# levi106/kvedge

Measured on AMD Instinct MI355X. Metric: images/sec ResNet-50 edge module at 1/2/4/8 MI355X; VM boot-to-ready sec, higher is better.
Workload: dtype bf16; 1 GPU; model=resnet50, global_batch=1280, per_gpu_batch=1280, image_size=224, parallelism=dp1, backend=none, hip_graph=True, streams=2, microbatch=0, mb_blocks=3

## Files before the change

### csrc/bindings/ops.cpp

```cpp
#include <ATen/ATen.h>
#include <c10/core/DeviceGuard.h>
#include <c10/hip/HIPStream.h>
#include <torch/library.h>

#include "../kernels/kvedge_kernels.h"

namespace {

hipStream_t cur_stream(const at::Tensor& t) {
  return c10::hip::getCurrentHIPStream(t.device().index()).stream();
}

void check_dev(const at::Tensor& t, const char* name) {
  TORCH_CHECK(t.is_cuda(), "kvedge: ", name, " must be a GPU tensor");
  TORCH_CHECK(t.is_contiguous(), "kvedge: ", name, " must be contiguous");
}

void check_bf16(const at::Tensor& t, const char* name) {
  check_dev(t, name);
  TORCH_CHECK(t.scalar_type() == at::kBFloat16, "kvedge: ", name, " must be bf16");
}

void set_splitk_ws(KvConvParams& p, const at::Tensor& ws) {
  p.ws = ws.data_ptr<float>();
// ... 78 lines not shown
  p.x = x.data_ptr();
  p.w = w.data_ptr();
  p.bias = bias.data_ptr<float>();
  p.N = (int)N; p.H = (int)H; p.W = (int)W; p.Cin = (int)Cin;
  p.ldx = (int)ldx; p.x_coff = (int)x_coff;
  p.Ho = (int)H; p.Wo = (int)W; p.Cout = (int)Cout;
  p.KH = 3; p.KW = 3; p.stride = 1; p.pad = 1;
  p.K = (int)(9 * Cin); p.Kpad = (int)w.size(1);
  p.M = (int)(N * H * W);
  p.act = (int)act; p.mode = 0;
  p.w_t = w2.data_ptr(); p.bias_t = b2.data_ptr<float>(); p.z = z.data_ptr();
  p.n_t = (int)C2; p.ldz = (int)z.size(3); p.z_coff = (int)z_coff;
  p.pair_1x1 = 1;
  const int rc = kv_conv_pair(&p, (int)tile, cur_stream(x));
  TORCH_CHECK(rc == 0, "kvedge: conv_pair failed rc=", rc);
}

void conv_dual(const at::Tensor& x1, const at::Tensor& x2, const at::Tensor& w,
               const c10::optional<at::Tensor>& bias, at::Tensor& y, int64_t stride2,
               int64_t act, int64_t tile, const c10::optional<at::Tensor>& ws) {
  check_bf16(x1, "x1");
  check_bf16(x2, "x2");
  check_bf16(w, "w");
  check_bf16(y, "y");
  TORCH_CHECK(x1.dim() == 4 && x2.dim() == 4 && y.dim() == 4, "kvedge: NHWC tensors");
  const int64_t N = x1.size(0), Ho = x1.size(1), Wo = x1.size(2), K1 = x1.size(3);
  const int64_t K2 = x2.size(3), Cout = y.size(3);
  TORCH_CHECK(x2.size(0) == N && (x2.size(1) + stride2 - 1) / stride2 == Ho &&
                  (x2.size(2) + stride2 - 1) / stride2 == Wo, "kvedge: x2 geometry vs stride");
  TORCH_CHECK(y.size(0) == N && y.size(1) == Ho && y.size(2) == Wo, "kvedge: y shape");
// ... 610 lines not shown
}

int64_t c2f16_supported(int64_t H, int64_t W, int64_t S) {
  return kv_c2f16_supported((int)H, (int)W, (int)S);
}

}

TORCH_LIBRARY(kvedge, m) {
  m.def("conv(Tensor x, Tensor w, Tensor? bias, Tensor? res, Tensor(a!) y, int N, int H, int W, "
        "int Cin, int ldx, int x_coff, int Ho, int Wo, int Cout, int KH, int KW, int stride, "
        "int pad, int K, int ldy, int y_coff, int ldr, int r_coff, int act, int mode, int tile, "
        "Tensor(b!)? ws=None) -> ()");
  m.def("conv_pair(Tensor x, Tensor w, Tensor bias, Tensor w2, Tensor b2, Tensor(a!) z, int Cin, "
        "int x_coff, int z_coff, int act, int tile) -> ()");
  m.def("conv_dual(Tensor x1, Tensor x2, Tensor w, Tensor? bias, Tensor(a!) y, int stride2, int act, "
        "int tile, Tensor(b!)? ws=None) -> ()");
  m.def("conv_tail(Tensor x, Tensor? x2, Tensor w, Tensor? bias, Tensor? res, Tensor(a!) y, "
        "Tensor w1, Tensor? b1, Tensor(b!) z, int stride2, int act, int tile) -> ()");
  m.def("conv_frames_s2d(Tensor frames, Tensor w, Tensor? bias, Tensor(a!) y, int act, "
        "int tile) -> ()");
  m.def("stem_pool(Tensor x, Tensor w, Tensor bias, Tensor(a!) y, int y_coff) -> ()");
  m.def("maxpool2d(Tensor x, Tensor(a!) y, int N, int H, int W, int C, int ldx, int x_coff, int ldy, "
        "int y_coff, int k, int stride, int pad, int Ho, int Wo) -> ()");
  m.def("sppf_pool(Tensor(a!) buf, int N, int H, int W, int C) -> ()");
  m.def("global_avgpool(Tensor x, Tensor(a!) y, int N, int HW, int C) -> ()");
  m.def("softmax_rows(Tensor x, Tensor(a!) y, Tensor(b!) argmax) -> ()");
  m.def("pooled_fc(Tensor x, Tensor w, Tensor? bias, Tensor(a!) y) -> ()");
  m.def("upsample2x(Tensor x, Tensor(a!) y, int N, int H, int W, int C, int ldx, int x_coff, int ldy, "
        "int y_coff) -> ()");
// ... 22 lines not shown
        "Tensor wm2, Tensor bm2, Tensor w2, Tensor b2, Tensor(a!) y, int y_coff, int S) -> ()");
  m.def("c2f16_supported(int H, int W, int S) -> int", c2f16_supported);
  m.def("conv_dual2(Tensor x, int x_coff, int K1, Tensor x2, int x2_coff, Tensor w, Tensor? bias, "
        "Tensor(a!) y, int y_coff, int stride2, int up2, int act, int tile, Tensor(b!)? ws=None) -> ()");
  m.def("set_conv_chunk_bytes(int bytes) -> int", set_conv_chunk_bytes);
}

TORCH_LIBRARY_IMPL(kvedge, CUDA, m) {
  m.impl("conv", conv);
  m.impl("conv_dual", conv_dual);
  m.impl("maxpool2d", maxpool2d);
  m.impl("stem_pool", stem_pool);
  m.impl("conv_frames_s2d", conv_frames_s2d);
  m.impl("conv_tail", conv_tail);
  m.impl("conv_pair", conv_pair);
  m.impl("c2f16_fused", c2f16_fused);
  m.impl("conv_dual2", conv_dual2);
  m.impl("sppf_pool", sppf_pool);
  m.impl("global_avgpool", global_avgpool);
  m.impl("softmax_rows", softmax_rows);
  m.impl("pooled_fc", pooled_fc);
  m.impl("upsample2x", upsample2x);
  m.impl("yolo_decode", yolo_decode);
  m.impl("nms", nms);
  m.impl("synth_frames", synth_frames);
  m.impl("synth_frames_dev", synth_frames_dev);
  m.impl("preprocess", preprocess);
  m.impl("stem_pool_frames", stem_pool_frames);
  m.impl("stem12_pool_frames", stem12_pool_frames);
  m.impl("yolo_stem2", yolo_stem2);
// ... 8 lines not shown
```

### csrc/kernels/conv_direct.hip

```cpp
#include <stdlib.h>
#include <string.h>

#include "common.h"
#include "kvedge_kernels.h"

typedef float floatx16 __attribute__((ext_vector_type(16)));

namespace kvedge {
namespace {

constexpr int kNT = 512;
constexpr int kOOB = 0x7ffffff0;
constexpr int kLds = 160 * 1024;
constexpr int kBiasBytes = 4 * 128;

template <int K>
__device__ __forceinline__ void direct_wait_vm_le_(int n) {
  if constexpr (K == 0) {
    asm volatile("s_waitcnt vmcnt(0)" ::: "memory");
  } else {
    if (n >= K) asm volatile("s_waitcnt vmcnt(%0)" ::"n"(K) : "memory");
    else direct_wait_vm_le_<K - 4>(n);
  }
}
// ... 8 lines not shown
  static constexpr int PRE = CIN >= 80 ? 6 : CIN >= 64 ? 7 : 10;
  static constexpr int MAX_PATCH = PRE * kNT * 16;
};

#ifndef KV_DIRECT_PD
#define KV_DIRECT_PD 8
#endif
constexpr int KPD = KV_DIRECT_PD;

__host__ __device__ constexpr int direct_patch_alloc(int patch_bytes, bool dma) {
  return dma ? (patch_bytes + 1023) / 1024 * 1024 : (patch_bytes + 15) / 16 * 16;
}

template <int CIN, int COUT, int S, int KK, int ACT, bool RES, bool U8 = false, bool DMA = false,
          bool PAIRS = false, int OCC = 1, int NT = kNT, int C2 = 0, bool DE = false,
          bool SB = false>
__global__ __launch_bounds__(NT, (NT / 256) * OCC) void conv3x3_direct_kernel(const KvConvParams p, int kR,
                                                                int PW, int patch_rows,
                                                                FastDiv fPW, FastDiv fWo,
                                                                int diag) {
  static_assert(!U8 || (CIN == 16 && KK == 2 && S == 1), "frames-in form: the 2x2 s2d stem");
  static_assert(!PAIRS || U8, "paired raw-row loads: frames-in form only");
  static_assert(KK != 1 || S == 1, "1x1 form: stride 1");
  constexpr int PADK = KK == 1 ? 0 : 1;
  using C = DirectCfg<CIN, KK>;
  constexpr int NCB = (COUT + 31) / 32;
  static_assert(NCB >= 1 && NCB <= 4 && NCB <= NT / 64, "channel blocks");
  constexpr int NPH = (NT / 64) / NCB;
  constexpr int OS = COUT + 8;
  static_assert(C2 == 0 || (!RES && !U8 && KK == 3 && COUT % 16 == 0), "pair form");
  constexpr int NCB2 = (C2 + 31) / 32;
  extern __shared__ __attribute__((aligned(16))) unsigned char lds[];
  static_assert(!(DMA && U8), "DMA patch fetch: bf16 NHWC inputs only");
  static_assert(!DE || (DMA && C2 == 0 && !U8 && !(RES && SB)), "direct epilogue: plain DMA forms");
  static_assert(!SB || DE, "single patch buffer: direct-epilogue forms");
  static_assert(!DE || COUT % 16 == 0, "direct epilogue: 16-channel store pairs");
  const int psz = direct_patch_alloc(patch_rows * PW * C::PB, DMA);
  unsigned char* patch = lds;
  bf16* otile = reinterpret_cast<bf16*>(lds + (DMA && !SB ? 2 * psz : psz));

  const int H = p.H, W = p.W, Ho = p.Ho, Wo = p.Wo;
  const int nbands = (Ho + kR - 1) / kR;
  const int total = p.N * nbands;
  const int tid = threadIdx.x, lane = tid & 63;
  const int wv = __builtin_amdgcn_readfirstlane(tid >> 6);
  const int fr = lane & 31, fh = lane >> 5;
  const int cb = wv % NCB, ph = wv / NCB;

  const bf16* wp = reinterpret_cast<const bf16*>(p.w);
  const int wrow = cb * 32 + fr;
  bf16x8 wreg[C::KS];
// ... 15 lines not shown
      for (int e = 0; e < 4; ++e) {
        const int c = cb * 32 + g * 8 + fh * 4 + e;
        breg[4 * g + e] = (p.bias && c < COUT) ? p.bias[c] : 0.f;
      }
  }
  float* lbias2 = lbias + 128;
  bf16* w2s = reinterpret_cast<bf16*>(lbias2 + 128);
  if constexpr (C2 > 0) {
    static_assert(NCB2 * 32 <= 128 && NCB * 32 <= 128, "pair bias slots");
    if (tid < NCB2 * 32) lbias2[tid] = (p.bias_t && tid < C2) ? p.bias_t[tid] : 0.f;
    const bf16* w2 = reinterpret_cast<const bf16*>(p.w_t);
    for (int q = tid; q < C2 * (COUT / 8); q += NT) {
      const int r = q / (COUT / 8), c = (q - r * (COUT / 8)) * 8;
      *reinterpret_cast<bf16x8*>(w2s + r * OS + c) =
          *reinterpret_cast<const bf16x8*>(w2 + (size_t)r * COUT + c);
    }
  }

  const int nchunks = patch_rows * PW * C::CPP;
  uint4 pre[C::PRE];
  const __amdgpu_buffer_rsrc_t rx = __builtin_amdgcn_make_buffer_rsrc(
      const_cast<void*>(p.x), (short)0, U8 ? p.N * H * W * 12 : p.N * H * W * p.ldx * 2,
      0x00020000);
  typedef unsigned int u32x4 __attribute__((ext_vector_type(4)));
  const int HALF = (PW + 1) >> 1;
  auto col_of = [&](int pos) __attribute__((always_inline)) {
    if constexpr (S == 2) return pos < HALF ? 2 * pos : 2 * (pos - HALF) + 1;
    return pos;
  };
  auto chunk_of = [&](int q, int& pp, int& c) __attribute__((always_inline)) {
// ... 143 lines not shown
  for (; item < total; item += gridDim.x) {
    const int n = item / nbands, band = item - n * nbands;
    const int oy0 = band * kR;
    if constexpr (SB) {
      dma_fetch(item, patch);
      asm volatile("s_waitcnt vmcnt(0)" ::: "memory");
      asm volatile("s_waitcnt lgkmcnt(0)" ::: "memory");
      __builtin_amdgcn_s_barrier();
      asm volatile("" ::: "memory");
    } else if constexpr (DMA) {
      if (!(DE && (diag & 2))) dma_fetch(item + gridDim.x, patch + (cur ^ 1) * psz);
    } else {
      fetch(item + gridDim.x);
    }
    const unsigned char* pbase = patch + cur * psz;
    constexpr int OCH = COUT / 8;
    constexpr int RPF = RES && !DE && CIN <= 32 ? (DMA ? 12 : CIN <= 16 ? 6 : 0) : 0;
    uint4 rpf[RPF > 0 ? RPF : 1];
    const bool rpre = RPF > 0 && npix * OCH <= RPF * NT;
    if constexpr (RPF > 0) {
      if (rpre) {
#pragma unroll
        for (int i = 0; i < RPF; ++i) {
          const int q = tid + NT * i;
          const int px = q / OCH, c = q - (q / OCH) * OCH;
          const int yl = fdiv(px, fWo), xc = px - yl * Wo;
          const int oy = oy0 + yl;
          rpf[i] = make_uint4(0u, 0u, 0u, 0u);
          if (q < npix * OCH && oy < Ho) {
            const long long m = (long long)(n * Ho + oy) * Wo + xc;
// ... 242 lines not shown

typedef void (*DirectFn)(const KvConvParams, int, int, int, FastDiv, FastDiv, int);

struct DirectEntry {
  int cin, cout, stride, kk, act;
  bool res;
  DirectFn fn;
  bool u8 = false;
  bool dma = false;
  bool pairs = false;
  int occ = 1;
  int nt = kNT;
  int c2 = 0;
  bool de = false;
  bool sb = false;
};

#define KV_DIRECT(CI, CO, S, A, R) {CI, CO, S, 3, A, R, conv3x3_direct_kernel<CI, CO, S, 3, A, R>}
#define KV_DIRECT_DMA(CI, CO, S, A, R) \
  {CI, CO, S, 3, A, R, conv3x3_direct_kernel<CI, CO, S, 3, A, R, false, true>, false, true}
#define KV_DIRECT2(CI, CO, S, A, R) KV_DIRECT(CI, CO, S, A, R), KV_DIRECT_DMA(CI, CO, S, A, R)
#define KV_DIRECT_OCC2(CI, CO, S, KK, A, R)                                                       \
  {CI, CO, S, KK, A, R, conv3x3_direct_kernel<CI, CO, S, KK, A, R, false, true, false, 2>, false, \
   true, false, 2}
#define KV_DIRECT_DE(CI, CO, S, KK, A)                                                          \
  {CI, CO, S, KK, A, false,                                                                    \
   conv3x3_direct_kernel<CI, CO, S, KK, A, false, false, true, false, 1, kNT, 0, true>, false,  \
   true, false, 1, kNT, 0, true}
#define KV_DIRECT_DER(CI, CO, OCC)                                                               \
  {CI, CO, 1, 3, kActSilu, true,                                                                 \
// ... 67 lines not shown
    KV_DIRECT_DE(192, 64, 1, 1, kActSilu), KV_DIRECT_DE(96, 64, 1, 1, kActSilu),
    KV_DIRECT_DE(64, 64, 1, 1, kActNone), KV_DIRECT_DE(80, 80, 1, 1, kActNone),
    KV_DIRECT_DE2(16, 32, 2, 3, kActSilu), KV_DIRECT_DE2(16, 16, 1, 3, kActSilu),
    KV_DIRECT_DE2(32, 64, 2, 3, kActSilu), KV_DIRECT_DE2(32, 32, 1, 3, kActSilu),
    KV_DIRECT_DE2(32, 32, 1, 1, kActSilu), KV_DIRECT_DE2(48, 32, 1, 1, kActSilu),
    KV_DIRECT_DER(16, 16, 1), KV_DIRECT_DER(32, 32, 1), KV_DIRECT_DER(64, 64, 1),
    KV_DIRECT_DER(16, 16, 2), KV_DIRECT_DER(32, 32, 2),
    KV_DIRECT_SB(64, 64, 1, 3, kActRelu), KV_DIRECT_SB(64, 128, 1, 3, kActSilu),
    KV_DIRECT_SB(64, 16, 1, 3, kActSilu), KV_DIRECT_SB(64, 64, 1, 3, kActSilu),
    KV_DIRECT_SB(64, 80, 1, 3, kActSilu),
    KV_DIRECT_SB(64, 128, 2, 3, kActSilu), KV_DIRECT_SB(64, 64, 2, 3, kActSilu),
    KV_DIRECT_SB(32, 64, 2, 3, kActSilu), KV_DIRECT_SB(32, 32, 1, 3, kActSilu),
    KV_DIRECT_SB(80, 80, 1, 3, kActSilu),
    KV_DIRECT_DE4(128, 128, 1, 3, kActRelu), KV_DIRECT_DE4(128, 128, 1, 3, kActSilu),
    KV_DIRECT_DE4(128, 128, 2, 3, kActSilu),
};
#undef KV_DIRECT2
#undef KV_DIRECT_DE
#undef KV_DIRECT_DE2
#undef KV_DIRECT_DER
#undef KV_DIRECT_SB
#undef KV_DIRECT_DE4
#undef KV_DIRECT1
#undef KV_DIRECT_OCC2
#undef KV_DIRECT_DMA
#undef KV_DIRECT

int direct_pb(int cin) { return cin * 2 + 16; }
int direct_max_patch(int cin) { return (cin >= 80 ? 6 : cin >= 64 ? 7 : 10) * kNT * 16; }

// ... 10 lines not shown
              : (p->mode != 0 || p->pad != 1))
    return -8;
  if (p->stride != 1 && p->stride != 2) return -8;
  if (kk == 2 && (p->stride != 1 || p->Ho != p->H || p->Wo != p->W)) return -8;
  const int act = p->act & 3;
  const bool res = p->res != nullptr;
  if (res && !(p->act & 4) && act != kActNone) return -8;
  int idx = -1;
  for (int pass = 0; pass < ((tile & 4) ? 1 : 2) && idx < 0; ++pass) {
    for (int i = 0; i < (int)(sizeof(kDirect) / sizeof(kDirect[0])); ++i) {
      const DirectEntry& e = kDirect[i];
      if (e.cin == p->Cin && e.cout == p->Cout && e.stride == p->stride && e.kk == kk &&
          e.act == act && e.res == res && e.u8 == (p->in_u8 != 0) &&
          (!e.u8 || e.pairs == (p->W % 2 == 0)) &&
          e.c2 == (p->pair_1x1 ? p->n_t : 0) && e.de == ((tile & 4) != 0) &&
          e.sb == ((tile & 8) != 0) &&
          (pass == 1 || (e.dma == ((tile & 1) != 0) && e.occ == 1 + ((tile >> 1) & 1)))) {
        idx = i;
        break;
      }
    }
  }
  if (idx < 0) return -8;
  if (p->Kpad != (kk * kk * p->Cin + 63) / 64 * 64 || p->ldx % 8 || p->x_coff % 8) return -8;
  if (p->in_u8 && (long long)p->N * p->H * p->W * 12 >= kOOB) return -9;
  if (kk == 3 && (p->Ho != (p->H - 1) / p->stride + 1 || p->Wo != (p->W - 1) / p->stride + 1))
    return -8;
  if (!p->in_u8 && (long long)p->N * p->H * p->W * p->ldx * 2 >= kOOB) return -9;
  if ((long long)p->N * p->Ho * p->Wo * p->ldy * 2 >= kOOB) return -9;
  if (p->pair_1x1 && (long long)p->N * p->Ho * p->Wo * p->ldz * 2 >= kOOB) return -9;
  if (res && (long long)p->N * p->Ho * p->Wo * p->ldr * 2 >= kOOB) return -9;
  const int S = p->stride;
  *PW = (p->Wo - 1) * S + kk;
  const int pb = direct_pb(p->Cin);
  const int os = p->Cout + 8;
  const bool dma = kDirect[idx].dma;
  auto lds_of = [&](int prows, int r) {
    const int np = dma && !kDirect[idx].sb ? 2 : 1;
    const int c2p = kDirect[idx].c2;
    const int ot = kDirect[idx].de ? 0 : ((r * p->Wo * os * 2 + 15) & ~15);
    return np * direct_patch_alloc(prows * *PW * pb, dma) + ot + kBiasBytes +
           (c2p ? kBiasBytes + c2p * os * 2 : 0);
  };
  int r = 8;
  for (; r >= 1; --r) {
    const int prows = (r - 1) * S + kk;
    const int patch = prows * *PW * pb;
    if ((dma || patch <= direct_max_patch(p->Cin)) && lds_of(prows, r) <= kLds / kDirect[idx].occ)
      break;
  }
  if (r < 1) return -11;
  if (r > p->Ho) r = p->Ho;
  *kR = r;
  *rows = (r - 1) * S + kk;
  *lds = lds_of(*rows, r);
  return idx;
}
// ... 15 lines not shown
  const long long slots = (long long)ncu * kDirect[idx].occ;
  const unsigned g = (unsigned)(items < slots ? items : slots);
  const DirectFn fn = kDirect[idx].fn;
  if (hipFuncSetAttribute(reinterpret_cast<const void*>(fn),
                          hipFuncAttributeMaxDynamicSharedMemorySize, lds) != hipSuccess)
    return -7;
  hipLaunchKernelGGL(fn, dim3(g), dim3(kDirect[idx].nt), (unsigned)lds, stream, *p, kR, PW, rows,
                     make_fastdiv(PW), make_fastdiv(p->Wo), direct_diag());
  return hipGetLastError() == hipSuccess ? 0 : -7;
}

int direct_launch(const KvConvParams* p, int tile, hipStream_t stream) {
  if (tile < 0 || tile >= 16) return -6;
  int kR, PW, rows, lds;
  if (direct_plan(p, tile, &kR, &PW, &rows, &lds) >= 0) return direct_launch_one(p, tile, stream);
  if (p->res || p->Cout % 16 || p->pair_1x1) return -8;
  static const bool greedy =
      !(getenv("KVEDGE_DIRECT_SPLIT") && strcmp(getenv("KVEDGE_DIRECT_SPLIT"), "balanced") == 0);
  int cuts[8], ncut = 0, done = 0;
  auto fits = [&](int cout) {
    KvConvParams q = *p;
    q.Cout = cout;
    return direct_plan(&q, tile, &kR, &PW, &rows, &lds) >= 0;
  };
  if (!greedy) {
    int best = 0;
    for (const DirectEntry& e : kDirect) {
      const int a = e.cout, b = p->Cout - e.cout;
      if (a >= b && b > 0 && (best == 0 || a < best) && fits(a) && fits(b)) best = a;
    }
    if (best) {
// ... 32 lines not shown
int direct_de_launch(const KvConvParams* p, int tile, hipStream_t stream) {
  if (tile < 0 || tile >= direct_de_num_tiles() || p->pair_1x1) return -8;
  static const bool de_res = !getenv("KVEDGE_DE_RES") || atoi(getenv("KVEDGE_DE_RES")) != 0;
  if (p->res && !de_res) return -8;
  static const int code[3] = {4 | 1, 4 | 2 | 1, 4 | 8 | 2 | 1};
  return direct_launch(p, code[tile], stream);
}

}

extern "C" int kv_conv_pair(const KvConvParams* p, int tile, hipStream_t stream) {
  if (!p->pair_1x1 || p->n_t <= 0 || !p->w_t || !p->z) return -8;
  return kvedge::direct_launch(p, tile, stream);
}
extern "C" int kv_conv_pair_num_tiles(void) { return kvedge::direct_num_tiles(); }
```

### csrc/kernels/conv_igemm.hip

```cpp
#include <algorithm>

#include "common.h"
#include "kvedge_kernels.h"

namespace kvedge {
namespace {

constexpr int BK = 64;

struct TileCfg {
  int bm, bn, wm, wn;
};

template <int BM, int BN, int WM, int WN, int MODE>
__global__ __launch_bounds__(256, 2) void conv_igemm_kernel(const KvConvParams p) {
  constexpr int WTM = BM / WM, WTN = BN / WN;
  constexpr int TM = WTM / 16, TN = WTN / 16;
  constexpr int AR = BM / 32;
  constexpr int BR = BN / 32;
  static_assert(WM * WN == 4, "4 waves per workgroup");
  static_assert(TM >= 1 && TN >= 1, "wave tile >= 16x16");

  __shared__ __attribute__((aligned(16))) bf16 smem[2 * (BM + BN) * BK];

// ... 361 lines not shown
  if (p->n_t) m = std::max(m, ohw * p->ldz * 2);
  return m;
}

static long long g_chunk_bytes = 0x7f000000LL;

extern "C" long long kv_set_conv_chunk_bytes(long long bytes) {
  g_chunk_bytes = bytes > 0 ? std::min(bytes, 0x7f000000LL) : 0x7f000000LL;
  return g_chunk_bytes;
}

extern "C" int kv_conv2d(const KvConvParams* p, int tile, hipStream_t stream) {
#ifdef KVEDGE_CHECKS
  if (const int rc = kv_conv_check_extents(p)) return rc;
#endif
  const long long kChunkBytes = g_chunk_bytes;
  const long long per = kv_conv_max_image_bytes(p);
  if (per <= 0 || per >= kChunkBytes) return per <= 0 ? -1 : -9;
  const long long cap = kChunkBytes / per;
  if (p->N <= cap) return kv_conv2d_one(p, tile, stream);
  const long long hw = (long long)p->H * p->W, ohw = (long long)p->Ho * p->Wo;
  for (int n0 = 0; n0 < p->N; n0 += (int)cap) {
    KvConvParams q = *p;
    q.N = (int)std::min<long long>(cap, p->N - n0);
    q.M = (int)(q.N * ohw);
    auto adv = [&](const void* b, long long bytes_per_image) -> const char* {
      return b ? static_cast<const char*>(b) + (long long)n0 * bytes_per_image : nullptr;
    };
    q.x = adv(p->x, p->in_u8 ? hw * 12 : hw * p->ldx * 2);
    q.y = const_cast<char*>(adv(p->y, ohw * p->ldy * 2));
// ... 70 lines not shown
```

### csrc/kernels/kvedge_kernels.h

```cpp
#pragma once
#include <hip/hip_runtime.h>
#include <stdint.h>

#ifdef __cplusplus
extern "C" {
#endif

typedef struct KvConvParams {
  const void* x;
  const void* w;
  const float* bias;
  const void* res;
  void* y;
  int N, H, W, Cin;
  int ldx, x_coff;
  int Ho, Wo, Cout;
  int KH, KW, stride, pad;
  int K, Kpad;
  int M;
  int ldy, y_coff, ldr, r_coff;
  int act;
  int mode;
  const void* x2;
  int K1, H2, W2, ldx2, stride2;
  int in_u8;
  const void* w_t;
  const float* bias_t;
  void* z;
  int n_t, ldz, z_coff, act_t;
  int pair_1x1;
  float* ws;
  int ksplit;
  long long ws_elems;
  int x2_coff;
  int up2;
} KvConvParams;

int kv_conv2d(const KvConvParams* p, int tile, hipStream_t stream);
long long kv_set_conv_chunk_bytes(long long bytes);
int kv_conv_num_tiles(void);
int kv_conv_splitk_base(void);
int kv_conv_splitk_num_tiles(void);
int kv_nloop_sched_check(void);
int kv_conv_pick_tile(const KvConvParams* p);
int kv_conv_seam_num_tiles(void);
int kv_conv_pair(const KvConvParams* p, int tile, hipStream_t stream);
int kv_conv_pair_num_tiles(void);

int kv_stem_pool(const void* x, const void* w, const float* bias, void* y, int N, int H, int W,
                 int ldy, int y_coff, hipStream_t s);
int kv_stem_pool_lds_bytes(int W);
int kv_stem_pool_frames(const void* frames, const void* w, const float* bias, void* y, int N,
                        int H0, int W0, const float* mean3, const float* inv_std3, int ldy,
                        int y_coff, hipStream_t s);
int kv_stem12_pool_frames(const void* frames, const void* w, const float* bias, void* y, int N,
                          int H0, int W0, const float* mean3, const float* inv_std3, int ldy,
                          int y_coff, hipStream_t s);
int kv_stem12_lds_bytes(int Ws);
int kv_yolo_stem2(const void* frames, const void* w0, const float* bias0, const void* w1,
                  int w1_ld, const float* bias1, void* y, int N, int H0, int W0, hipStream_t s);
int kv_yolo_stem2_lds_bytes(int Ws);

// ... 56 lines not shown
```

### kvedge_amd/engine/profile.py

```python
from __future__ import annotations

import contextlib
import functools
import json
from typing import Dict, List

import torch

from .. import ops

_OPS = ("conv2d", "conv_dual", "conv_dual2", "conv_tail", "conv_pair", "c2f16", "stem_pool",
        "stem_pool_frames", "stem12_pool_frames", "stem_from_frames", "yolo_stem2", "maxpool2d",
        "sppf_pool", "global_avgpool", "pooled_fc", "softmax_rows", "upsample2x", "yolo_decode",
        "nms", "synth_frames", "preprocess", "batchnorm_nhwc", "frame_resize", "det_to_source",
        "roi_crop")


def _shape_of(out):
    if isinstance(out, torch.Tensor):
        return list(out.shape)
    if isinstance(out, (tuple, list)) and out and isinstance(out[0], torch.Tensor):
        return list(out[0].shape)
    return None


@contextlib.contextmanager
# ... 56 lines not shown
```

### kvedge_amd/models/resnet.py

```python
from __future__ import annotations

import os

from typing import List, Optional

import torch
import torch.nn as nn
import torch.nn.functional as F

from .. import ops
from .layers import (DeployedConv, DeployedDualConv, calibrate_bn, count_flops, fold_bn,
                     frames_to_nchw)

ACT_NONE, ACT_RELU = ops.ACT_NONE, ops.ACT_RELU
TAIL1_MIN_ROWS = int(os.environ.get("KVEDGE_TAIL1_MIN_ROWS", "32768"))


class Bottleneck(nn.Module):
    expansion = 4

    def __init__(self, cin: int, width: int, stride: int):
        super().__init__()
        cout = width * self.expansion
        self.conv1 = nn.Conv2d(cin, width, 1, bias=False)
        self.bn1 = nn.BatchNorm2d(width)
        self.conv2 = nn.Conv2d(width, width, 3, stride, 1, bias=False)
        self.bn2 = nn.BatchNorm2d(width)
        self.conv3 = nn.Conv2d(width, cout, 1, bias=False)
        self.bn3 = nn.BatchNorm2d(cout)
        self.downsample = None
# ... 47 lines not shown
            nn.init.ones_(mod.weight)
            nn.init.zeros_(mod.bias)
        elif isinstance(mod, nn.Linear):
            bound = 1.0 / mod.in_features ** 0.5
            with torch.no_grad():
                mod.weight.uniform_(-bound, bound, generator=g)
                mod.bias.uniform_(-bound, bound, generator=g)
    if calibrate:
        frames = torch.randint(0, 256, (calib_batch, calib_hw, calib_hw, 3), generator=g,
                               dtype=torch.uint8)
        calibrate_bn(m, [frames_to_nchw(frames)])
    m.eval()
    return m


class DeployedBottleneck:

    def __init__(self, b: Bottleneck, device, fuse_down: bool = True):
        self.c1 = DeployedConv.from_modules(b.conv1, b.bn1, ACT_RELU, device)
        self.c2 = DeployedConv.from_modules(b.conv2, b.bn2, ACT_RELU, device)
        self.c3 = DeployedConv.from_modules(b.conv3, b.bn3, ACT_RELU, device)
        self.down = None
        self.dual = None
        if b.downsample is not None:
            self.down = DeployedConv.from_modules(b.downsample[0], b.downsample[1], ACT_NONE,
                                                  device)
            if fuse_down:
                self.dual = DeployedDualConv.from_modules(b.conv3, b.bn3, b.downsample[0],
                                                          b.downsample[1], ACT_RELU, device)

    def __call__(self, x, out=None, t1=None):
        y = self.c1(x) if t1 is None else t1
        y = self.c2(y)
        if self.dual is not None:
            return self.dual(y, x, out=out)
        idt = x if self.down is None else self.down(x)
        return self.c3(y, res=idt, out=out)

    def can_tail(self, nxt: "DeployedBottleneck") -> bool:
        c1 = nxt.c1.spec
        cout = self.c3.spec.cout
        if not (c1.kh == 1 and c1.stride == 1 and c1.pad == 0 and c1.cin == cout and
                c1.act == ACT_RELU and self.c3.spec.act == ACT_RELU):
            return False
        if cout != 256:
            k3 = self.c3.spec.cin
            return (ops.SEAM_ENABLED and self.down is None and self.dual is None and
                    (k3, cout, c1.cout) in ops.SEAM_SHAPES)
        k = self.c3.spec.cin + (self.dual.w.shape[1] - self.dual.k1 if self.dual is not None else 0)
        return (c1.cout in (64, 128) and (self.dual is not None or self.down is None) and
                (self.dual is None or c1.cout == 64) and k <= 128)

    def tail_fits(self, x: torch.Tensor, batch: int = 0) -> bool:
        N, Ho, Wo, _ = self.out_shape(x.shape)
        N = batch or N
        if self.c3.spec.cout == 256:
            return N * Ho * Wo >= TAIL1_MIN_ROWS
        return (N * Ho * Wo + 127) // 128 >= ops.SEAM_MIN_WGS

    def call_tail(self, x, nxt: "DeployedBottleneck", t1=None, out=None, z=None):
        y = self.c1(x) if t1 is None else t1
        y = self.c2(y)
        c1 = nxt.c1
        if self.dual is not None:
            d = self.dual
            return ops.conv_tail(y, d.w, d.b, d.act, c1.w, c1.b, x2=x, stride2=d.stride2,
                                 out=out, z=z)
        return ops.conv_tail(y, self.c3.w, self.c3.b, self.c3.spec.act, c1.w, c1.b, res=x,
                             out=out, z=z)

    def out_shape(self, x_shape):
        N, H, W, _ = x_shape
        Ho, Wo = self.c2.spec.out_hw(H, W)
        return (N, Ho, Wo, self.c3.spec.cout)

    def convs(self):
        return [c for c in (self.c1, self.c2, self.c3, self.down, self.dual) if c is not None]
# ... 68 lines not shown
                z = None
                for j in range(nb):
                    b, nxt = self.blocks[j], self.blocks[j + 1]
                    last = j == nb - 1
                    if last and full is None:
                        shp = b.out_shape(y.shape)
                        full = ops.empty((B,) + shp[1:], dtype=y.dtype, device=y.device)
                    fuse = (self.fuse_tail and y.is_cuda and b.can_tail(nxt) and
                            b.tail_fits(y, batch=B))
                    if last and full_t1 is None and fuse:
                        full_t1 = ops.empty(full.shape[:3] + (nxt.c1.spec.cout,),
                                            dtype=y.dtype, device=y.device)
                    o = full[i:i + mb] if last else None
                    if fuse:
                        y, z = b.call_tail(y, nxt, t1=z, out=o,
                                           z=full_t1[i:i + mb] if last else None)
                    else:
                        y, z = b(y, t1=z, out=o), None
            x, t1 = full, full_t1
            rest = self.blocks[nb:]
        else:
            x = self.stem_and_pool(x, frames_in)
            rest = self.blocks
        for i, b in enumerate(rest):
            nxt = rest[i + 1] if i + 1 < len(rest) else None
            if (self.fuse_tail and x.is_cuda and nxt is not None and b.can_tail(nxt) and
                    b.tail_fits(x)):
                x, t1 = b.call_tail(x, nxt, t1=t1)
            else:
                x, t1 = b(x, t1=t1), None
        return x

    def logits(self, x: torch.Tensor, frames_in: bool = False) -> torch.Tensor:
# ... 19 lines not shown
```

### kvedge_amd/ops/__init__.py

```python
from __future__ import annotations

import os
from dataclasses import dataclass
from typing import Optional, Sequence, Tuple

import torch

from . import reference as _ref

_LIB_PATH = os.path.join(os.path.dirname(os.path.dirname(os.path.abspath(__file__))),
                         "_C_checks.so" if os.environ.get("KVEDGE_CHECKS", "0") not in ("", "0")
                         else os.path.basename(os.environ.get("KVEDGE_LIB", "") or "_C.so"))
_loaded = False
_load_error: Optional[str] = None

ACT_NONE, ACT_RELU, ACT_SILU = 0, 1, 2
RES_AFTER_ACT = 4
MODE_GENERAL, MODE_GEMM, MODE_STEM = 0, 1, 2
BK = 64


def load(build_if_missing: bool = False) -> bool:
    global _loaded, _load_error
    if _loaded:
# ... 183 lines not shown
              w2: torch.Tensor, b2: torch.Tensor, out: torch.Tensor, x_coff: int = 0,
              z_coff: int = 0, tile: int = 0) -> torch.Tensor:
    assert spec.kh == 3 and spec.stride == 1 and spec.pad == 1 and spec.mode == MODE_GENERAL
    C2 = w2.shape[0]
    assert w2.shape[1] == spec.cout and out.shape[:3] == x.shape[:3]
    if x.is_cuda:
        _native().conv_pair(x, w, bias, w2, b2, out, spec.cin, x_coff, z_coff, spec.act, tile)
        return out
    t = torch.empty(*x.shape[:3], spec.cout, dtype=torch.bfloat16)
    _ref.conv2d(x, spec, w, bias, None, t, x_coff, 0, 0)
    z = t.float() @ w2.float().t() + b2.float()
    out[..., z_coff:z_coff + C2] = z.to(out.dtype)
    return out


def conv_dual(x1: torch.Tensor, x2: torch.Tensor, w: torch.Tensor, bias: Optional[torch.Tensor],
              act: int, stride2: int, out: Optional[torch.Tensor] = None,
              tile: int = -1) -> torch.Tensor:
    N, Ho, Wo, K1 = x1.shape
    cout = w.shape[0]
    if out is None:
        out = empty(N, Ho, Wo, cout, dtype=torch.bfloat16, device=x1.device)
    if x1.is_cuda:
        ws = splitk_workspace(x1.device, N * Ho * Wo * cout) if is_splitk(tile) else None
        _native().conv_dual(x1, x2, w, bias, out, stride2, act, tile, ws)
    else:
        _ref.conv_dual(x1, x2, w, bias, act, stride2, out)
    return out


# ... 458 lines not shown
```

Baseline: 86430 images/sec.

## Fuse leading 1x1 conv into direct 3x3 conv patch load for ResNet 64-channel blocks

```diff
diff --git a/csrc/bindings/ops.cpp b/csrc/bindings/ops.cpp
--- a/csrc/bindings/ops.cpp
+++ b/csrc/bindings/ops.cpp
@@ -116,6 +116,48 @@
   p.pair_1x1 = 1;
   const int rc = kv_conv_pair(&p, (int)tile, cur_stream(x));
   TORCH_CHECK(rc == 0, "kvedge: conv_pair failed rc=", rc);
+}
+
+void conv_pre1x1(const at::Tensor& x, const at::Tensor& w1, const at::Tensor& b1,
+                 const at::Tensor& w, const at::Tensor& bias, at::Tensor& y, int64_t act,
+                 int64_t tile) {
+  check_bf16(x, "x");
+  check_bf16(w1, "w1");
+  check_bf16(w, "w");
+  check_bf16(y, "y");
+  check_dev(b1, "b1");
+  check_dev(bias, "bias");
+  TORCH_CHECK(x.dim() == 4 && y.dim() == 4 && w.dim() == 2 && w1.dim() == 2, "kvedge: conv_pre1x1 shapes");
+  const int64_t N = x.size(0), H = x.size(1), W = x.size(2), Cin0 = x.size(3);
+  const int64_t Cin = w1.size(0), Cout = w.size(0);
+  TORCH_CHECK(N > 0 && H > 0 && W > 0, "kvedge: conv_pre1x1 empty input");
+  TORCH_CHECK(w1.size(1) == (Cin0 + 63) / 64 * 64 && Cin0 % 8 == 0,
+              "kvedge: conv_pre1x1 w1 must be the packed [Cin, Kpad(Cin0)]");
+  TORCH_CHECK(w.size(1) == (9 * Cin + 63) / 64 * 64, "kvedge: conv_pre1x1 w must be [Cout, Kpad(9 Cin)]");
+  TORCH_CHECK(y.size(0) == N && y.size(1) == H && y.size(2) == W && y.size(3) == Cout,
+              "kvedge: conv_pre1x1 y [N, H, W, Cout]");
+  TORCH_CHECK(b1.scalar_type() == at::kFloat && b1.numel() >= Cin && bias.scalar_type() == at::kFloat &&
+              bias.numel() >= Cout, "kvedge: conv_pre1x1 biases fp32");
+  TORCH_CHECK(N * H * W * Cin0 * 2 < (1ll << 31) && N * H * W * Cout * 2 < (1ll << 31),
+              "kvedge: conv_pre1x1 operands exceed 2 GiB");
+  const c10::DeviceGuard g(x.device());
+  KvConvParams p{};
+  p.x = x.data_ptr();
+  p.w = w.data_ptr();
+  p.bias = bias.data_ptr<float>();
+  p.y = y.data_ptr();
+  p.N = (int)N; p.H = (int)H; p.W = (int)W; p.Cin = (int)Cin;
+  p.ldx = (int)Cin0; p.x_coff = 0;
+  p.Ho = (int)H; p.Wo = (int)W; p.Cout = (int)Cout;
+  p.KH = 3; p.KW = 3; p.stride = 1; p.pad = 1;
+  p.K = (int)(9 * Cin); p.Kpad = (int)w.size(1);
+  p.M = (int)(N * H * W);
+  p.ldy = (int)Cout; p.y_coff = 0;
+  p.act = (int)act; p.mode = 0;
+  p.w_t = w1.data_ptr(); p.bias_t = b1.data_ptr<float>(); p.n_t = (int)Cin0;
+  p.pre_1x1 = 1;
+  const int rc = kv_conv_pre1x1(&p, (int)tile, cur_stream(x));
+  TORCH_CHECK(rc == 0, "kvedge: conv_pre1x1 failed rc=", rc);
 }
 
 void conv_dual(const at::Tensor& x1, const at::Tensor& x2, const at::Tensor& w,
@@ -756,6 +798,8 @@
         "Tensor(b!)? ws=None) -> ()");
   m.def("conv_pair(Tensor x, Tensor w, Tensor bias, Tensor w2, Tensor b2, Tensor(a!) z, int Cin, "
         "int x_coff, int z_coff, int act, int tile) -> ()");
+  m.def("conv_pre1x1(Tensor x, Tensor w1, Tensor b1, Tensor w, Tensor bias, Tensor(a!) y, int act, "
+        "int tile) -> ()");
   m.def("conv_dual(Tensor x1, Tensor x2, Tensor w, Tensor? bias, Tensor(a!) y, int stride2, int act, "
         "int tile, Tensor(b!)? ws=None) -> ()");
   m.def("conv_tail(Tensor x, Tensor? x2, Tensor w, Tensor? bias, Tensor? res, Tensor(a!) y, "
@@ -808,6 +852,7 @@
   m.impl("conv_frames_s2d", conv_frames_s2d);
   m.impl("conv_tail", conv_tail);
   m.impl("conv_pair", conv_pair);
+  m.impl("conv_pre1x1", conv_pre1x1);
   m.impl("c2f16_fused", c2f16_fused);
   m.impl("conv_dual2", conv_dual2);
   m.impl("sppf_pool", sppf_pool);
diff --git a/csrc/kernels/conv_direct.hip b/csrc/kernels/conv_direct.hip
--- a/csrc/kernels/conv_direct.hip
+++ b/csrc/kernels/conv_direct.hip
@@ -46,7 +46,7 @@
 
 template <int CIN, int COUT, int S, int KK, int ACT, bool RES, bool U8 = false, bool DMA = false,
           bool PAIRS = false, int OCC = 1, int NT = kNT, int C2 = 0, bool DE = false,
-          bool SB = false>
+          bool SB = false, bool PRE = false>
 __global__ __launch_bounds__(NT, (NT / 256) * OCC) void conv3x3_direct_kernel(const KvConvParams p, int kR,
                                                                 int PW, int patch_rows,
                                                                 FastDiv fPW, FastDiv fWo,
@@ -67,6 +67,8 @@
   static_assert(!DE || (DMA && C2 == 0 && !U8 && !(RES && SB)), "direct epilogue: plain DMA forms");
   static_assert(!SB || DE, "single patch buffer: direct-epilogue forms");
   static_assert(!DE || COUT % 16 == 0, "direct epilogue: 16-channel store pairs");
+  static_assert(!PRE || (DE && !RES && CIN == 64 && KK == 3 && S == 1),
+                "pre-1x1: 64 -> 64 in front of a stride-1 3x3, direct-epilogue forms");
   const int psz = direct_patch_alloc(patch_rows * PW * C::PB, DMA);
   unsigned char* patch = lds;
   bf16* otile = reinterpret_cast<bf16*>(lds + (DMA && !SB ? 2 * psz : psz));
@@ -112,6 +114,18 @@
       const int r = q / (COUT / 8), c = (q - r * (COUT / 8)) * 8;
       *reinterpret_cast<bf16x8*>(w2s + r * OS + c) =
           *reinterpret_cast<const bf16x8*>(w2 + (size_t)r * COUT + c);
+    }
+  }
+
+  float* lb1 = lbias + 128;
+  unsigned char* w1s = reinterpret_cast<unsigned char*>(lb1 + 128);
+  if constexpr (PRE) {
+    if (tid < CIN) lb1[tid] = p.bias_t ? p.bias_t[tid] : 0.f;
+    const bf16* w1 = reinterpret_cast<const bf16*>(p.w_t);
+    for (int q = tid; q < CIN * C::CPP; q += NT) {
+      const int r = q / C::CPP, c = q - r * C::CPP;
+      *reinterpret_cast<uint4*>(w1s + r * C::PB + c * 16) =
+          *reinterpret_cast<const uint4*>(w1 + r * CIN + c * 8);
     }
   }
 
@@ -285,6 +299,78 @@
       fetch(item + gridDim.x);
     }
     const unsigned char* pbase = patch + cur * psz;
+    if constexpr (PRE) {
+      typedef unsigned int u32x2 __attribute__((ext_vector_type(2)));
+      const int np = patch_rows * PW;
+      const int iy0 = oy0 - 1;
+      unsigned char* pw = patch + cur * psz;
+      const unsigned wa = lds_addr(w1s + fr * C::PB + fh * 16);
+      for (int g = wv; g * 32 < np; g += NT / 64) {
+        const int pp = g * 32 + fr;
+        const int pq = min(pp, np - 1);
+        const int pr = fdiv(pq, fPW), pc = pq - pr * PW;
+        const bool inimg = pp < np && (unsigned)(iy0 + pr) < (unsigned)H &&
+                           (unsigned)(pc - 1) < (unsigned)W;
+        unsigned char* px = pw + pq * C::PB;
+        const unsigned xa = lds_addr(px + fh * 16);
+        constexpr int PT = NT == kNT ? 2 : 3;
+        constexpr int NS = PT + 1;
+        static_assert(C::KPT == 4 && PT < C::KPT, "pre-1x1: K = 64 in four steps");
+        floatx4 bq[8];
+        bf16x8 fx[NS], f0[NS], f1[NS];
+        const unsigned ba1 = lds_addr(lb1 + fh * 4);
+        auto rd3 = [&](auto kc) __attribute__((always_inline)) {
+          constexpr int k = decltype(kc)::value;
+          lds_read16<k * 32>(fx[k % NS], xa);
+          lds_read16<k * 32>(f0[k % NS], wa);
+          lds_read16<32 * C::PB + k * 32>(f1[k % NS], wa);
+        };
+        static_range<0, PT>(rd3);
+        floatx16 a0 = {}, a1 = {};
+        static_range<0, C::KPT>([&](auto kc) __attribute__((always_inline)) {
+          constexpr int k = decltype(kc)::value;
+          constexpr int issued = k + PT < C::KPT ? k + PT : C::KPT;
+          asm volatile("s_waitcnt lgkmcnt(%3)"
+                       : "+v"(fx[k % NS]), "+v"(f0[k % NS]), "+v"(f1[k % NS])
+                       : "n"(3 * (issued - k - 1))
+                       : "memory");
+          if constexpr (k + PT < C::KPT) rd3(IC<k + PT>{});
+          if constexpr (k == C::KPT - 1)
+            static_range<0, 4>([&](auto gc) __attribute__((always_inline)) {
+              constexpr int gq = decltype(gc)::value;
+              lds_read16<gq * 32>(bq[gq], ba1);
+              lds_read16<128 + gq * 32>(bq[4 + gq], ba1);
+            });
+          a0 = __builtin_amdgcn_mfma_f32_32x32x16_bf16(f0[k % NS], fx[k % NS], a0, 0, 0, 0);
+          a1 = __builtin_amdgcn_mfma_f32_32x32x16_bf16(f1[k % NS], fx[k % NS], a1, 0, 0, 0);
+        });
+        asm volatile("s_waitcnt lgkmcnt(0)"
+                     : "+v"(bq[0]), "+v"(bq[1]), "+v"(bq[2]), "+v"(bq[3]), "+v"(bq[4]),
+                       "+v"(bq[5]), "+v"(bq[6]), "+v"(bq[7])::"memory");
+#pragma unroll
+        for (int hb = 0; hb < 2; ++hb) {
+          const floatx16& a = hb ? a1 : a0;
+#pragma unroll
+          for (int q = 0; q < 2; ++q) {
+            bf16x4 lo, hi;
+#pragma unroll
+            for (int e = 0; e < 4; ++e) {
+              lo[e] = f2bf(fmaxf(a[8 * q + e] + bq[4 * hb + 2 * q][e], 0.f));
+              hi[e] = f2bf(fmaxf(a[8 * q + 4 + e] + bq[4 * hb + 2 * q + 1][e], 0.f));
+            }
+            const u32x2 b0 = __builtin_bit_cast(u32x2, lo), b1 = __builtin_bit_cast(u32x2, hi);
+            const auto s0 = __builtin_amdgcn_permlane32_swap(b0[0], b1[0], false, false);
+            const auto s1 = __builtin_amdgcn_permlane32_swap(b0[1], b1[1], false, false);
+            if (inimg)
+              *reinterpret_cast<uint4*>(px + hb * 64 + q * 32 + fh * 16) =
+                  make_uint4(s0[0], s1[0], s0[1], s1[1]);
+          }
+        }
+      }
+      asm volatile("s_waitcnt lgkmcnt(0)" ::: "memory");
+      __builtin_amdgcn_s_barrier();
+      asm volatile("" ::: "memory");
+    }
     constexpr int OCH = COUT / 8;
     constexpr int RPF = RES && !DE && CIN <= 32 ? (DMA ? 12 : CIN <= 16 ? 6 : 0) : 0;
     uint4 rpf[RPF > 0 ? RPF : 1];
@@ -557,6 +643,7 @@
   int c2 = 0;
   bool de = false;
   bool sb = false;
+  bool pre = false;
 };
 
 #define KV_DIRECT(CI, CO, S, A, R) {CI, CO, S, 3, A, R, conv3x3_direct_kernel<CI, CO, S, 3, A, R>}
@@ -654,6 +741,14 @@
     KV_DIRECT_SB(80, 80, 1, 3, kActSilu),
     KV_DIRECT_DE4(128, 128, 1, 3, kActRelu), KV_DIRECT_DE4(128, 128, 1, 3, kActSilu),
     KV_DIRECT_DE4(128, 128, 2, 3, kActSilu),
+    {64, 64, 1, 3, kActRelu, false,
+     conv3x3_direct_kernel<64, 64, 1, 3, kActRelu, false, false, true, false, 1, kNT, 0, true, false,
+                           true>,
+     false, true, false, 1, kNT, 0, true, false, true},
+    {64, 64, 1, 3, kActRelu, false,
+     conv3x3_direct_kernel<64, 64, 1, 3, kActRelu, false, false, true, false, 2, 256, 0, true, true,
+                           true>,
+     false, true, false, 2, 256, 0, true, true, true},
 };
 #undef KV_DIRECT2
 #undef KV_DIRECT_DE
@@ -694,7 +789,7 @@
           e.act == act && e.res == res && e.u8 == (p->in_u8 != 0) &&
           (!e.u8 || e.pairs == (p->W % 2 == 0)) &&
           e.c2 == (p->pair_1x1 ? p->n_t : 0) && e.de == ((tile & 4) != 0) &&
-          e.sb == ((tile & 8) != 0) &&
+          e.sb == ((tile & 8) != 0) && e.pre == (p->pre_1x1 != 0) &&
           (pass == 1 || (e.dma == ((tile & 1) != 0) && e.occ == 1 + ((tile >> 1) & 1)))) {
         idx = i;
         break;
@@ -720,7 +815,8 @@
     const int c2p = kDirect[idx].c2;
     const int ot = kDirect[idx].de ? 0 : ((r * p->Wo * os * 2 + 15) & ~15);
     return np * direct_patch_alloc(prows * *PW * pb, dma) + ot + kBiasBytes +
-           (c2p ? kBiasBytes + c2p * os * 2 : 0);
+           (c2p ? kBiasBytes + c2p * os * 2 : 0) +
+           (kDirect[idx].pre ? kBiasBytes + p->Cin * pb : 0);
   };
   int r = 8;
   for (; r >= 1; --r) {
@@ -766,7 +862,7 @@
   if (tile < 0 || tile >= 16) return -6;
   int kR, PW, rows, lds;
   if (direct_plan(p, tile, &kR, &PW, &rows, &lds) >= 0) return direct_launch_one(p, tile, stream);
-  if (p->res || p->Cout % 16 || p->pair_1x1) return -8;
+  if (p->res || p->Cout % 16 || p->pair_1x1 || p->pre_1x1) return -8;
   static const bool greedy =
       !(getenv("KVEDGE_DIRECT_SPLIT") && strcmp(getenv("KVEDGE_DIRECT_SPLIT"), "balanced") == 0);
   int cuts[8], ncut = 0, done = 0;
@@ -829,3 +925,8 @@
   return kvedge::direct_launch(p, tile, stream);
 }
 extern "C" int kv_conv_pair_num_tiles(void) { return kvedge::direct_num_tiles(); }
+extern "C" int kv_conv_pre1x1(const KvConvParams* p, int tile, hipStream_t stream) {
+  if (!p->pre_1x1 || p->n_t != p->Cin || !p->w_t || p->res || p->pair_1x1) return -8;
+  return kvedge::direct_de_launch(p, tile, stream);
+}
+extern "C" int kv_conv_pre1x1_num_tiles(void) { return kvedge::direct_de_num_tiles(); }
diff --git a/csrc/kernels/conv_igemm.hip b/csrc/kernels/conv_igemm.hip
--- a/csrc/kernels/conv_igemm.hip
+++ b/csrc/kernels/conv_igemm.hip
@@ -399,6 +399,7 @@
 #ifdef KVEDGE_CHECKS
   if (const int rc = kv_conv_check_extents(p)) return rc;
 #endif
+  if (p->pre_1x1) return -8;
   const long long kChunkBytes = g_chunk_bytes;
   const long long per = kv_conv_max_image_bytes(p);
   if (per <= 0 || per >= kChunkBytes) return per <= 0 ? -1 : -9;
diff --git a/csrc/kernels/kvedge_kernels.h b/csrc/kernels/kvedge_kernels.h
--- a/csrc/kernels/kvedge_kernels.h
+++ b/csrc/kernels/kvedge_kernels.h
@@ -34,6 +34,7 @@
   long long ws_elems;
   int x2_coff;
   int up2;
+  int pre_1x1;
 } KvConvParams;
 
 int kv_conv2d(const KvConvParams* p, int tile, hipStream_t stream);
@@ -46,6 +47,8 @@
 int kv_conv_seam_num_tiles(void);
 int kv_conv_pair(const KvConvParams* p, int tile, hipStream_t stream);
 int kv_conv_pair_num_tiles(void);
+int kv_conv_pre1x1(const KvConvParams* p, int tile, hipStream_t stream);
+int kv_conv_pre1x1_num_tiles(void);
 
 int kv_stem_pool(const void* x, const void* w, const float* bias, void* y, int N, int H, int W,
                  int ldy, int y_coff, hipStream_t s);
diff --git a/kvedge_amd/engine/profile.py b/kvedge_amd/engine/profile.py
--- a/kvedge_amd/engine/profile.py
+++ b/kvedge_amd/engine/profile.py
@@ -9,7 +9,8 @@
 
 from .. import ops
 
-_OPS = ("conv2d", "conv_dual", "conv_dual2", "conv_tail", "conv_pair", "c2f16", "stem_pool",
+_OPS = ("conv2d", "conv_dual", "conv_dual2", "conv_tail", "conv_pair", "conv_pre1x1", "c2f16",
+        "stem_pool",
         "stem_pool_frames", "stem12_pool_frames", "stem_from_frames", "yolo_stem2", "maxpool2d",
         "sppf_pool", "global_avgpool", "pooled_fc", "softmax_rows", "upsample2x", "yolo_decode",
         "nms", "synth_frames", "preprocess", "batchnorm_nhwc", "frame_resize", "det_to_source",
diff --git a/kvedge_amd/models/resnet.py b/kvedge_amd/models/resnet.py
--- a/kvedge_amd/models/resnet.py
+++ b/kvedge_amd/models/resnet.py
@@ -9,11 +9,12 @@
 import torch.nn.functional as F
 
 from .. import ops
-from .layers import (DeployedConv, DeployedDualConv, calibrate_bn, count_flops, fold_bn,
-                     frames_to_nchw)
+from .layers import (DeployedConv, DeployedDualConv, _record, _recorder_active, calibrate_bn,
+                     count_flops, fold_bn, frames_to_nchw)
 
 ACT_NONE, ACT_RELU = ops.ACT_NONE, ops.ACT_RELU
 TAIL1_MIN_ROWS = int(os.environ.get("KVEDGE_TAIL1_MIN_ROWS", "32768"))
+PRE1X1_MIN_ROWS = int(os.environ.get("KVEDGE_PRE1X1_MIN_ROWS", "32768"))
 
 
 class Bottleneck(nn.Module):
@@ -91,6 +92,24 @@
     return m
 
 
+class DeployedPre1x1:
+
+    def __init__(self, c1: DeployedConv, c2: DeployedConv):
+        self.c1, self.c2 = c1, c2
+        self.tile = ops.PRE1X1_TILES[0]
+
+    def __call__(self, x, out=None, tile=None):
+        c1, c2 = self.c1, self.c2
+        out = ops.conv_pre1x1(x, c1.w, c1.b, c2.spec, c2.w, c2.b, out=out,
+                              tile=self.tile if tile is None else tile)
+        if _recorder_active():
+            key = ("pre1x1", c1.spec.cin, c2.spec.cin, c2.spec.cout, tuple(x.shape))
+            fn = lambda t, o=out: ops.conv_pre1x1(x, c1.w, c1.b, c2.spec, c2.w,
+                                                  c2.b, out=o, tile=t)
+            _record(self, key, fn)
+        return out
+
+
 class DeployedBottleneck:
 
     def __init__(self, b: Bottleneck, device, fuse_down: bool = True):
@@ -99,6 +118,8 @@
         self.c3 = DeployedConv.from_modules(b.conv3, b.bn3, ACT_RELU, device)
         self.down = None
         self.dual = None
+        self.pre = (DeployedPre1x1(self.c1, self.c2)
+                    if ops.pre1x1_eligible(self.c1.spec, self.c2.spec) else None)
         if b.downsample is not None:
             self.down = DeployedConv.from_modules(b.downsample[0], b.downsample[1], ACT_NONE,
                                                   device)
@@ -106,9 +127,17 @@
                 self.dual = DeployedDualConv.from_modules(b.conv3, b.bn3, b.downsample[0],
                                                           b.downsample[1], ACT_RELU, device)
 
-    def __call__(self, x, out=None, t1=None):
-        y = self.c1(x) if t1 is None else t1
-        y = self.c2(y)
+    def c12(self, x, t1=None, batch: int = 0):
+        if t1 is not None:
+            return self.c2(t1)
+        N, H, W, _ = x.shape
+        if (self.pre is not None and x.is_cuda and ops.PRE1X1_ENABLED and
+                (batch or N) * H * W >= PRE1X1_MIN_ROWS):
+            return self.pre(x)
+        return self.c2(self.c1(x))
+
+    def __call__(self, x, out=None, t1=None, batch: int = 0):
+        y = self.c12(x, t1, batch)
         if self.dual is not None:
             return self.dual(y, x, out=out)
         idt = x if self.down is None else self.down(x)
@@ -135,9 +164,8 @@
             return N * Ho * Wo >= TAIL1_MIN_ROWS
         return (N * Ho * Wo + 127) // 128 >= ops.SEAM_MIN_WGS
 
-    def call_tail(self, x, nxt: "DeployedBottleneck", t1=None, out=None, z=None):
-        y = self.c1(x) if t1 is None else t1
-        y = self.c2(y)
+    def call_tail(self, x, nxt: "DeployedBottleneck", t1=None, out=None, z=None, batch: int = 0):
+        y = self.c12(x, t1, batch)
         c1 = nxt.c1
         if self.dual is not None:
             d = self.dual
@@ -236,9 +264,9 @@
                     o = full[i:i + mb] if last else None
                     if fuse:
                         y, z = b.call_tail(y, nxt, t1=z, out=o,
-                                           z=full_t1[i:i + mb] if last else None)
+                                           z=full_t1[i:i + mb] if last else None, batch=B)
                     else:
-                        y, z = b(y, t1=z, out=o), None
+                        y, z = b(y, t1=z, out=o, batch=B), None
             x, t1 = full, full_t1
             rest = self.blocks[nb:]
         else:
diff --git a/kvedge_amd/ops/__init__.py b/kvedge_amd/ops/__init__.py
--- a/kvedge_amd/ops/__init__.py
+++ b/kvedge_amd/ops/__init__.py
@@ -221,6 +221,37 @@
     return out
 
 
+PRE1X1_ENABLED = os.environ.get("KVEDGE_PRE1X1", "1") != "0"
+PRE1X1_TILES = (0, 2)
+
+
+def pre1x1_eligible(s1: ConvSpec, s2: ConvSpec) -> bool:
+    return (s1.kh == 1 and s1.kw == 1 and s1.stride == 1 and s1.pad == 0 and
+            s1.act == ACT_RELU and s1.mode == MODE_GEMM and
+            s2.kh == 3 and s2.kw == 3 and s2.stride == 1 and s2.pad == 1 and s2.pad_end == 1 and
+            s2.act == ACT_RELU and s2.mode == MODE_GENERAL and
+            (s1.cin, s1.cout, s2.cin, s2.cout) == (64, 64, 64, 64))
+
+
+def conv_pre1x1(x: torch.Tensor, w1: torch.Tensor, b1: torch.Tensor, spec: ConvSpec,
+                w: torch.Tensor, bias: torch.Tensor, out: Optional[torch.Tensor] = None,
+                tile: int = 0) -> torch.Tensor:
+    assert spec.kh == 3 and spec.stride == 1 and spec.pad == 1 and spec.mode == MODE_GENERAL
+    N, H, W, cin0 = x.shape
+    s1 = ConvSpec.auto(cin0, spec.cin, 1, 1, 0, ACT_RELU)
+    assert w1.shape == (spec.cin, s1.Kpad), (w1.shape, spec.cin, s1.Kpad)
+    if out is None:
+        out = empty(N, H, W, spec.cout, dtype=torch.bfloat16, device=x.device)
+    assert out.shape == (N, H, W, spec.cout), (out.shape, (N, H, W, spec.cout))
+    if x.is_cuda:
+        _native().conv_pre1x1(x, w1, b1, w, bias, out, spec.act, tile)
+        return out
+    t = torch.empty(N, H, W, spec.cin, dtype=torch.bfloat16)
+    _ref.conv2d(x, s1, w1, b1, None, t, 0, 0, 0)
+    _ref.conv2d(t, spec, w, bias, None, out, 0, 0, 0)
+    return out
+
+
 def conv_dual(x1: torch.Tensor, x2: torch.Tensor, w: torch.Tensor, bias: Optional[torch.Tensor],
               act: int, stride2: int, out: Optional[torch.Tensor] = None,
               tile: int = -1) -> torch.Tensor:
```

Measured after the change: 87120 images/sec, median of 6. About the same (+0.8%).
